# rainerzufalldererste/limg

Measured on AMD Instinct MI355X. Metric: encode Mpixels/s, 8K RGBA (limg_encode3d_test-equivalent: all 11 planes stored), higher is better.
Workload: dtype u8/i32 integer stage + f32 float stage (bit-exact vs the reference's strict SSE build)

## Files before the change

limg_amd/csrc/limg_hip_search.h:

```cpp
#ifndef LIMG_HIP_SEARCH_H
#define LIMG_HIP_SEARCH_H

#include "limg_hip_device.h"
#include "limg_search_table.h"

namespace limg_hip
{
  namespace
  {
    struct __attribute__((aligned(32))) SearchEntry { uint32_t w[8]; };
    __constant__ SearchEntry d_search_tab[LIMG_SEARCH_STATES] = LIMG_SEARCH_TABLE_INIT;

    typedef short short2_t __attribute__((ext_vector_type(2)));
    typedef unsigned short ushort2_t __attribute__((ext_vector_type(2)));
    __device__ __forceinline__ constexpr int term_bias(int factor) { return factor == 2 ? 0x2000 : 0x3000; }
    __device__ __forceinline__ int term_const(int f, int c, int lo) { return 255 - ((lo << 8) + 128) + (c < 2 ? (term_bias(f) << 8) : 0); }

    struct TrialState
    {
      uint32_t fA, fB, fC;
      uint32_t loRG, hiRG;
      int pxB, pxBlo;
      int nA[3], nB[3], nC[3];
      int mA[3], mB[3], mC[3];
      uint32_t tA_RG, tB_RG, tC_RG;
      int tA_B, tB_B, tC_B;
      uint32_t cA, cB, cC;
    };

    __device__ __forceinline__ void make_terms(const uint32_t f, const uint32_t s, const uint32_t mul, const int n[3], const int m[3], uint32_t &tRG, int &tB)
    {
      const int d = (int)mul_u24_uniform(f >> (s & 31u), mul);
      const int t0 = mad_i24(d, n[0], m[0]), t1 = mad_i24(d, n[1], m[1]), t2 = mad_i24(d, n[2], m[2]);
      tRG = __builtin_amdgcn_perm((uint32_t)t1, (uint32_t)t0, 0x06050201u);
      tB = t2 >> 8;
    }

    __device__ __forceinline__ void rebuild_A(TrialState &t, const uint32_t sA, const uint32_t mul) { make_terms(t.fA, sA, mul, t.nA, t.mA, t.tA_RG, t.tA_B); t.cA = sA; }
    __device__ __forceinline__ void rebuild_B(TrialState &t, const uint32_t sB, const uint32_t mul)
    {
      if (sB > 7) { t.tB_RG = (uint32_t)term_bias(1) * 0x10001u; t.tB_B = 0; }
      else make_terms(t.fB, sB, mul, t.nB, t.mB, t.tB_RG, t.tB_B);
      t.cB = sB;
    }
    __device__ __forceinline__ void rebuild_C(TrialState &t, const uint32_t sC, const uint32_t mul)
    {
      if (sC > 7) { t.tC_RG = (uint32_t)term_bias(2) * 0x10001u; t.tC_B = 0; }
      else make_terms(t.fC, sC, mul, t.nC, t.mC, t.tC_RG, t.tC_B);
      t.cC = sC;
    }

    template <bool FULL>
    __device__ __forceinline__ uint32_t trial_pixel_error(const TrialState &t, const bool active)
    {
      const uint32_t dRG = t.tA_RG + t.tB_RG + t.tC_RG;
      const int dBraw = t.tA_B + t.tB_B + t.tC_B;
      ushort2_t eu = __builtin_bit_cast(ushort2_t, dRG);
      eu = __builtin_elementwise_max(eu, __builtin_bit_cast(ushort2_t, t.loRG));
      eu = __builtin_elementwise_min(eu, __builtin_bit_cast(ushort2_t, t.hiRG));
      int dB = med3_i32(dBraw, t.pxBlo, t.pxB);
      const ushort2_t sq = eu * eu;
      const uint32_t sqB = (uint32_t)mul_i24(dB, dB);
      const bool low_red = sq.x < 0x4000;
      const uint32_t half = __builtin_amdgcn_udot2(sq, __builtin_bit_cast(ushort2_t, 0x00020001u), sqB, false);
      const uint32_t extra = low_red ? sqB : (__builtin_bit_cast(uint32_t, sq) & 0xFFFFu);
      uint32_t err = (half << 1) + extra;
      if (!FULL) err = active ? err : 0u;
      return err;
    }

    typedef unsigned int uint8s_t __attribute__((ext_vector_type(8)));
    __device__ __forceinline__ uint8s_t sload8(const SearchEntry *base, uint32_t byteOffset)
    {
      uint8s_t v;
      asm volatile("s_load_dwordx8 %0, %1, %2\n\ts_waitcnt lgkmcnt(0)" : "=&s"(v) : "s"(base), "s"(byteOffset) : "memory");
      return v;
    }

    template <bool FULL>
    __device__ __forceinline__ void search_fast_automaton(TrialState &t, const bool active, const uint32_t maxPixel32, const uint32_t blockLimit, uint32_t shift[3])
    {
      const SearchEntry *tab = d_search_tab;
      asm volatile("" : "+s"(tab));
      constexpr uint32_t root[8] = LIMG_SEARCH_ROOT;
      rebuild_A(t, root[0] & 31u, root[5]);
      rebuild_B(t, root[3], root[6]);
      rebuild_C(t, root[4], root[7]);
      uint8s_t e = { root[0] & ~0xE0u, root[1], root[2], root[3], root[4], root[5], root[6], root[7] };
      while (!(e[0] >> 31))
      {
        if (e[0] & 0x20u) rebuild_A(t, e[0] & 31u, e[5]);
        if (e[0] & 0x40u) rebuild_B(t, e[3], e[6]);
        if (e[0] & 0x80u) rebuild_C(t, e[4], e[7]);
        const uint32_t err = trial_pixel_error<FULL>(t, active);
        uint32_t off;
        if (__builtin_amdgcn_ballot_w64(err > maxPixel32) != 0ull) off = e[2];
        else off = (wave_sum(err) < blockLimit) ? e[1] : e[2];
        e = sload8(tab, off);
      }
      shift[0] = e[0] & 31u; shift[1] = e[3]; shift[2] = e[4];
    }

    template <bool FULL>
    __device__ __forceinline__ void search_accurate_automaton(TrialState &t, const bool active, const uint32_t maxPixel32, const uint32_t blockLimit, const uint32_t *table,
                                                              uint32_t shift[3])
    {
      const SearchEntry *tab = reinterpret_cast<const SearchEntry *>(table);
      uint32_t bestA = 0, bestB = 0, bestC = 0, minBe = 0xFFFFFFFFu;
      {
        constexpr uint32_t root[8] = LIMG_SEARCH_ROOT;
        rebuild_A(t, root[0] & 31u, root[5]);
        rebuild_B(t, root[3], root[6]);
        rebuild_C(t, root[4], root[7]);
      }
      uint8s_t e = sload8(tab, 0u);
      constexpr uint32_t rootT[8] = LIMG_SEARCH_ROOT;
      uint32_t mask = ((e[0] & 31u) != (rootT[0] & 31u) ? 1u : 0u) | (e[3] != rootT[3] ? 2u : 0u) | (e[4] != rootT[4] ? 4u : 0u);
      while (!(e[0] >> 31))
      {
        const uint32_t a = e[0] & 31u;
        if (mask & 1u) rebuild_A(t, a, e[5]);
        if (mask & 2u) rebuild_B(t, e[3], e[6]);
        if (mask & 4u) rebuild_C(t, e[4], e[7]);
        const uint32_t err = trial_pixel_error<FULL>(t, active);
        uint32_t off = e[2];
        if (__builtin_amdgcn_ballot_w64(err > maxPixel32) == 0ull)
        {
          const uint32_t be = wave_sum(err);
          if (be < blockLimit)
          {
            off = e[1];
            if (!(e[0] & 0x20u) || be < minBe) { bestA = a; bestB = e[3]; bestC = e[4]; minBe = be; }
          }
        }
        mask = off >> 24;
        e = sload8(tab, off & 0xFFFFFFu);
      }
      shift[0] = bestA; shift[1] = bestB; shift[2] = bestC;
    }

    __device__ __attribute__((noinline)) uint32_t search_generic(uint32_t px, uint32_t fA, uint32_t fB, uint32_t fC, const int16_t *rec , bool active,
                                                                 uint32_t maxPixel32, uint64_t maxBlockN, bool fast)
    {
      RecU r;
#pragma unroll
      for (int c = 0; c < 3; c++)
      {
        const int loA = rec[c], hiA = rec[4 + c], loB = rec[8 + c], hiB = rec[12 + c], loC = rec[16 + c], hiC = rec[20 + c];
        r.nA[c] = sgpr(hiA - loA); r.nB[c] = sgpr(hiB - loB); r.nC[c] = sgpr(hiC - loC);
        r.mA[c] = sgpr((int)(((uint32_t)loA << 8) + 128u)); r.mB[c] = sgpr((int)(((uint32_t)loB << 8) + 128u)); r.mC[c] = sgpr((int)(((uint32_t)loC << 8) + 128u));
      }
      uint32_t shift[3] = { 0, 0, 0 };
      auto T = [&](uint32_t a, uint32_t bb, uint32_t c, uint32_t &be2) -> bool { return trial(px, fA, fB, fC, r, a, bb, c, active, maxPixel32, maxBlockN, be2); };
      if (fast) search_fast(T, shift);
      else search_accurate(T, shift);
      return shift[0] | (shift[1] << 8) | (shift[2] << 16);
    }
  }
}

#endif
```

Before: 51070.

## Unroll hot top of fast search automaton into compile-time branch tree

```diff
diff --git a/limg_amd/csrc/limg_hip_search.h b/limg_amd/csrc/limg_hip_search.h
--- a/limg_amd/csrc/limg_hip_search.h
+++ b/limg_amd/csrc/limg_hip_search.h
@@ -77,16 +77,55 @@
       return v;
     }
 
+    struct TermSet { uint32_t rg; int b; };
+    __device__ __forceinline__ constexpr TermSet terms_shift8(int factor) { return TermSet{ (uint32_t)term_bias(factor) * 0x10001u, 0 }; }
+    template <uint32_t S, uint32_t MUL>
+    __device__ __forceinline__ TermSet hot_terms(const uint32_t f, const int n[3], const int m[3])
+    {
+      static_assert(S <= 8 && (S >= 4 || MUL == (1u << S)), "MUL is shift_mul(S)");
+      int t0, t1, t2;
+      if constexpr (S == 8) { t0 = m[0]; t1 = m[1]; t2 = m[2]; }
+      else
+      {
+        uint32_t d;
+        if constexpr (S < 4) d = f & ~((1u << S) - 1u);
+        else asm("v_mul_u32_u24 %0, %2, %1" : "=v"(d) : "v"(f >> S), "n"(MUL));
+        t0 = mad_i24((int)d, n[0], m[0]); t1 = mad_i24((int)d, n[1], m[1]); t2 = mad_i24((int)d, n[2], m[2]);
+      }
+      TermSet r;
+      r.rg = __builtin_amdgcn_perm((uint32_t)t1, (uint32_t)t0, 0x06050201u);
+      r.b = t2 >> 8;
+      return r;
+    }
+    __device__ __forceinline__ bool hot_trial(TrialState &t, const TermSet &A, const TermSet &B, const TermSet &C, const uint32_t maxPixel32, const uint32_t blockLimit)
+    {
+      t.tA_RG = A.rg; t.tA_B = A.b; t.tB_RG = B.rg; t.tB_B = B.b; t.tC_RG = C.rg; t.tC_B = C.b;
+      const uint32_t err = trial_pixel_error<true>(t, true);
+      return __builtin_amdgcn_ballot_w64(err > maxPixel32) == 0ull && wave_sum(err) < blockLimit;
+    }
+#include "limg_search_hot.h"
+
     template <bool FULL>
     __device__ __forceinline__ void search_fast_automaton(TrialState &t, const bool active, const uint32_t maxPixel32, const uint32_t blockLimit, uint32_t shift[3])
     {
       const SearchEntry *tab = d_search_tab;
-      asm volatile("" : "+s"(tab));
-      constexpr uint32_t root[8] = LIMG_SEARCH_ROOT;
-      rebuild_A(t, root[0] & 31u, root[5]);
-      rebuild_B(t, root[3], root[6]);
-      rebuild_C(t, root[4], root[7]);
-      uint8s_t e = { root[0] & ~0xE0u, root[1], root[2], root[3], root[4], root[5], root[6], root[7] };
+      uint8s_t e;
+      if constexpr (FULL)
+      {
+        uint32_t off;
+        if (search_hot(t, maxPixel32, blockLimit, shift, off)) return;
+        asm volatile("" : "+s"(tab));
+        e = sload8(tab, off);
+      }
+      else
+      {
+        asm volatile("" : "+s"(tab));
+        constexpr uint32_t root[8] = LIMG_SEARCH_ROOT;
+        rebuild_A(t, root[0] & 31u, root[5]);
+        rebuild_B(t, root[3], root[6]);
+        rebuild_C(t, root[4], root[7]);
+        e = uint8s_t{ root[0] & ~0xE0u, root[1], root[2], root[3], root[4], root[5], root[6], root[7] };
+      }
       while (!(e[0] >> 31))
       {
         if (e[0] & 0x20u) rebuild_A(t, e[0] & 31u, e[5]);
diff --git a/limg_amd/csrc/limg_search_hot.h b/limg_amd/csrc/limg_search_hot.h
--- /dev/null
+++ b/limg_amd/csrc/limg_search_hot.h
@@ -0,0 +1,260 @@
+#ifndef LIMG_SEARCH_HOT_H
+#define LIMG_SEARCH_HOT_H
+#define LIMG_SEARCH_HOT_STATES 45
+__device__ __forceinline__ bool search_hot(TrialState &t, const uint32_t maxPixel32, const uint32_t blockLimit, uint32_t shift[3], uint32_t &off)
+{
+  const TermSet tA4_0 = hot_terms<4u, 17u>(t.fA, t.nA, t.mA);
+  const TermSet tB5_0 = hot_terms<5u, 36u>(t.fB, t.nB, t.mB);
+  const TermSet tC6_0 = hot_terms<6u, 85u>(t.fC, t.nC, t.mC);
+  if (hot_trial(t, tA4_0, tB5_0, tC6_0, maxPixel32, blockLimit))
+  {
+    const TermSet tA5_1 = hot_terms<5u, 36u>(t.fA, t.nA, t.mA);
+    if (hot_trial(t, tA5_1, terms_shift8(1), terms_shift8(2), maxPixel32, blockLimit))
+    { shift[0] = 5u; shift[1] = 8u; shift[2] = 8u; return true; }
+    else
+    {
+      const TermSet tB6_3 = hot_terms<6u, 85u>(t.fB, t.nB, t.mB);
+      if (hot_trial(t, tA4_0, tB6_3, terms_shift8(2), maxPixel32, blockLimit))
+      {
+        if (hot_trial(t, tA4_0, terms_shift8(1), terms_shift8(2), maxPixel32, blockLimit))
+        { t.cA = 4u; t.cB = 8u; t.cC = 8u; off = 0x00a0u; return false; }
+        else
+        {
+          const TermSet tA6_23 = hot_terms<6u, 85u>(t.fA, t.nA, t.mA);
+          if (hot_trial(t, tA6_23, tB6_3, terms_shift8(2), maxPixel32, blockLimit))
+          {
+            if (hot_trial(t, tA6_23, terms_shift8(1), terms_shift8(2), maxPixel32, blockLimit))
+            { t.cA = 6u; t.cB = 8u; t.cC = 8u; off = 0x00c0u; return false; }
+            else
+            {
+              const TermSet tA8_25 = hot_terms<8u, 256u>(t.fA, t.nA, t.mA);
+              if (hot_trial(t, tA8_25, tB6_3, terms_shift8(2), maxPixel32, blockLimit))
+              { t.cA = 8u; t.cB = 6u; t.cC = 8u; off = 0x0180u; return false; }
+              else
+              {
+                if (hot_trial(t, tA8_25, terms_shift8(1), tC6_0, maxPixel32, blockLimit))
+                { t.cA = 8u; t.cB = 8u; t.cC = 6u; off = 0x0220u; return false; }
+                else
+                {
+                  const TermSet tB7_27 = hot_terms<7u, 255u>(t.fB, t.nB, t.mB);
+                  if (hot_trial(t, tA6_23, tB7_27, terms_shift8(2), maxPixel32, blockLimit))
+                  { t.cA = 6u; t.cB = 7u; t.cC = 8u; off = 0x0380u; return false; }
+                  else
+                  {
+                    const TermSet tA7_31 = hot_terms<7u, 255u>(t.fA, t.nA, t.mA);
+                    if (hot_trial(t, tA7_31, tB6_3, terms_shift8(2), maxPixel32, blockLimit))
+                    { t.cA = 7u; t.cB = 6u; t.cC = 8u; off = 0x0400u; return false; }
+                    else
+                    { shift[0] = 6u; shift[1] = 6u; shift[2] = 8u; return true; }
+                  }
+                }
+              }
+            }
+          }
+          else
+          {
+            if (hot_trial(t, tA6_23, terms_shift8(1), tC6_0, maxPixel32, blockLimit))
+            { t.cA = 6u; t.cB = 8u; t.cC = 6u; off = 0x0480u; return false; }
+            else
+            {
+              const TermSet tA8_47 = hot_terms<8u, 256u>(t.fA, t.nA, t.mA);
+              if (hot_trial(t, tA8_47, tB6_3, terms_shift8(2), maxPixel32, blockLimit))
+              { t.cA = 8u; t.cB = 6u; t.cC = 8u; off = 0x0180u; return false; }
+              else
+              {
+                if (hot_trial(t, tA8_47, terms_shift8(1), tC6_0, maxPixel32, blockLimit))
+                { t.cA = 8u; t.cB = 8u; t.cC = 6u; off = 0x0220u; return false; }
+                else
+                {
+                  const TermSet tB7_49 = hot_terms<7u, 255u>(t.fB, t.nB, t.mB);
+                  if (hot_trial(t, tA4_0, tB7_49, terms_shift8(2), maxPixel32, blockLimit))
+                  { t.cA = 4u; t.cB = 7u; t.cC = 8u; off = 0x0640u; return false; }
+                  else
+                  {
+                    if (hot_trial(t, tA5_1, tB6_3, terms_shift8(2), maxPixel32, blockLimit))
+                    {
+                      if (hot_trial(t, tA5_1, tB7_49, terms_shift8(2), maxPixel32, blockLimit))
+                      { shift[0] = 5u; shift[1] = 7u; shift[2] = 8u; return true; }
+                      else
+                      { shift[0] = 5u; shift[1] = 6u; shift[2] = 8u; return true; }
+                    }
+                    else
+                    { shift[0] = 4u; shift[1] = 6u; shift[2] = 8u; return true; }
+                  }
+                }
+              }
+            }
+          }
+        }
+      }
+      else
+      {
+        if (hot_trial(t, tA4_0, tB5_0, terms_shift8(2), maxPixel32, blockLimit))
+        { t.cA = 4u; t.cB = 5u; t.cC = 8u; off = 0x0740u; return false; }
+        else
+        {
+          const TermSet tB7_96 = hot_terms<7u, 255u>(t.fB, t.nB, t.mB);
+          const TermSet tC5_96 = hot_terms<5u, 36u>(t.fC, t.nC, t.mC);
+          if (hot_trial(t, tA4_0, tB7_96, tC5_96, maxPixel32, blockLimit))
+          { t.cA = 4u; t.cB = 7u; t.cC = 5u; off = 0x0c20u; return false; }
+          else
+          {
+            const TermSet tA6_112 = hot_terms<6u, 85u>(t.fA, t.nA, t.mA);
+            const TermSet tB4_112 = hot_terms<4u, 17u>(t.fB, t.nB, t.mB);
+            const TermSet tC7_112 = hot_terms<7u, 255u>(t.fC, t.nC, t.mC);
+            if (hot_trial(t, tA6_112, tB4_112, tC7_112, maxPixel32, blockLimit))
+            { t.cA = 6u; t.cB = 4u; t.cC = 7u; off = 0x0c60u; return false; }
+            else
+            {
+              const TermSet tC4_113 = hot_terms<4u, 17u>(t.fC, t.nC, t.mC);
+              if (hot_trial(t, tA6_112, tB6_3, tC4_113, maxPixel32, blockLimit))
+              { t.cA = 6u; t.cB = 6u; t.cC = 4u; off = 0x0e40u; return false; }
+              else
+              {
+                if (hot_trial(t, tA6_112, terms_shift8(1), tC6_0, maxPixel32, blockLimit))
+                { t.cA = 6u; t.cB = 8u; t.cC = 6u; off = 0x0480u; return false; }
+                else
+                {
+                  const TermSet tA8_138 = hot_terms<8u, 256u>(t.fA, t.nA, t.mA);
+                  if (hot_trial(t, tA8_138, tB6_3, terms_shift8(2), maxPixel32, blockLimit))
+                  { t.cA = 8u; t.cB = 6u; t.cC = 8u; off = 0x0180u; return false; }
+                  else
+                  {
+                    if (hot_trial(t, tA8_138, terms_shift8(1), tC6_0, maxPixel32, blockLimit))
+                    { t.cA = 8u; t.cB = 8u; t.cC = 6u; off = 0x0220u; return false; }
+                    else
+                    {
+                      if (hot_trial(t, tA4_0, tB5_0, tC7_112, maxPixel32, blockLimit))
+                      { t.cA = 4u; t.cB = 5u; t.cC = 7u; off = 0x11a0u; return false; }
+                      else
+                      {
+                        if (hot_trial(t, tA5_1, tB5_0, tC6_0, maxPixel32, blockLimit))
+                        {
+                          if (hot_trial(t, tA5_1, tB5_0, tC7_112, maxPixel32, blockLimit))
+                          { shift[0] = 5u; shift[1] = 5u; shift[2] = 7u; return true; }
+                          else
+                          { shift[0] = 5u; shift[1] = 5u; shift[2] = 6u; return true; }
+                        }
+                        else
+                        { shift[0] = 4u; shift[1] = 5u; shift[2] = 6u; return true; }
+                      }
+                    }
+                  }
+                }
+              }
+            }
+          }
+        }
+      }
+    }
+  }
+  else
+  {
+    const TermSet tA2_148 = hot_terms<2u, 4u>(t.fA, t.nA, t.mA);
+    const TermSet tB4_148 = hot_terms<4u, 17u>(t.fB, t.nB, t.mB);
+    const TermSet tC5_148 = hot_terms<5u, 36u>(t.fC, t.nC, t.mC);
+    if (hot_trial(t, tA2_148, tB4_148, tC5_148, maxPixel32, blockLimit))
+    {
+      const TermSet tC7_149 = hot_terms<7u, 255u>(t.fC, t.nC, t.mC);
+      if (hot_trial(t, tA2_148, tB4_148, tC7_149, maxPixel32, blockLimit))
+      { t.cA = 2u; t.cB = 4u; t.cC = 7u; off = 0x12c0u; return false; }
+      else
+      {
+        const TermSet tB6_378 = hot_terms<6u, 85u>(t.fB, t.nB, t.mB);
+        const TermSet tC4_378 = hot_terms<4u, 17u>(t.fC, t.nC, t.mC);
+        if (hot_trial(t, tA2_148, tB6_378, tC4_378, maxPixel32, blockLimit))
+        { t.cA = 2u; t.cB = 6u; t.cC = 4u; off = 0x2f60u; return false; }
+        else
+        {
+          if (hot_trial(t, tA2_148, terms_shift8(1), tC6_0, maxPixel32, blockLimit))
+          { t.cA = 2u; t.cB = 8u; t.cC = 6u; off = 0x18e0u; return false; }
+          else
+          {
+            const TermSet tB2_412 = hot_terms<2u, 4u>(t.fB, t.nB, t.mB);
+            if (hot_trial(t, tA4_0, tB2_412, terms_shift8(2), maxPixel32, blockLimit))
+            { t.cA = 4u; t.cB = 2u; t.cC = 8u; off = 0x2500u; return false; }
+            else
+            {
+              if (hot_trial(t, tA4_0, tB4_148, tC4_378, maxPixel32, blockLimit))
+              {
+                if (hot_trial(t, tA4_0, tB4_148, tC6_0, maxPixel32, blockLimit))
+                { t.cA = 4u; t.cB = 4u; t.cC = 6u; off = 0x2700u; return false; }
+                else
+                {
+                  if (hot_trial(t, tA4_0, tB6_378, tC4_378, maxPixel32, blockLimit))
+                  { t.cA = 4u; t.cB = 6u; t.cC = 4u; off = 0x2a40u; return false; }
+                  else
+                  {
+                    if (hot_trial(t, tA4_0, terms_shift8(1), tC6_0, maxPixel32, blockLimit))
+                    { t.cA = 4u; t.cB = 8u; t.cC = 6u; off = 0x1460u; return false; }
+                    else
+                    {
+                      const TermSet tA6_417 = hot_terms<6u, 85u>(t.fA, t.nA, t.mA);
+                      if (hot_trial(t, tA6_417, tB4_148, terms_shift8(2), maxPixel32, blockLimit))
+                      { t.cA = 6u; t.cB = 4u; t.cC = 8u; off = 0x1620u; return false; }
+                      else
+                      {
+                        if (hot_trial(t, tA6_417, tB6_378, tC4_378, maxPixel32, blockLimit))
+                        { t.cA = 6u; t.cB = 6u; t.cC = 4u; off = 0x0e40u; return false; }
+                        else
+                        {
+                          if (hot_trial(t, tA6_417, terms_shift8(1), tC6_0, maxPixel32, blockLimit))
+                          { t.cA = 6u; t.cB = 8u; t.cC = 6u; off = 0x0480u; return false; }
+                          else
+                          {
+                            const TermSet tA8_420 = hot_terms<8u, 256u>(t.fA, t.nA, t.mA);
+                            if (hot_trial(t, tA8_420, tB6_378, terms_shift8(2), maxPixel32, blockLimit))
+                            { t.cA = 8u; t.cB = 6u; t.cC = 8u; off = 0x0180u; return false; }
+                            else
+                            {
+                              if (hot_trial(t, tA8_420, terms_shift8(1), tC6_0, maxPixel32, blockLimit))
+                              { t.cA = 8u; t.cB = 8u; t.cC = 6u; off = 0x0220u; return false; }
+                              else
+                              {
+                                if (hot_trial(t, tA4_0, tB4_148, tC5_148, maxPixel32, blockLimit))
+                                {
+                                  if (hot_trial(t, tA4_0, tB5_0, tC5_148, maxPixel32, blockLimit))
+                                  {
+                                    const TermSet tA5_424 = hot_terms<5u, 36u>(t.fA, t.nA, t.mA);
+                                    if (hot_trial(t, tA5_424, tB5_0, tC5_148, maxPixel32, blockLimit))
+                                    { shift[0] = 5u; shift[1] = 5u; shift[2] = 5u; return true; }
+                                    else
+                                    { shift[0] = 4u; shift[1] = 5u; shift[2] = 5u; return true; }
+                                  }
+                                  else
+                                  {
+                                    const TermSet tA5_427 = hot_terms<5u, 36u>(t.fA, t.nA, t.mA);
+                                    if (hot_trial(t, tA5_427, tB4_148, tC5_148, maxPixel32, blockLimit))
+                                    { t.cA = 5u; t.cB = 4u; t.cC = 5u; off = 0x3580u; return false; }
+                                    else
+                                    {
+                                      if (hot_trial(t, tA5_427, tB5_0, tC4_378, maxPixel32, blockLimit))
+                                      { t.cA = 5u; t.cB = 5u; t.cC = 4u; off = 0x35e0u; return false; }
+                                      else
+                                      { shift[0] = 4u; shift[1] = 4u; shift[2] = 5u; return true; }
+                                    }
+                                  }
+                                }
+                                else
+                                { t.cA = 4u; t.cB = 4u; t.cC = 5u; off = 0x3640u; return false; }
+                              }
+                            }
+                          }
+                        }
+                      }
+                    }
+                  }
+                }
+              }
+              else
+              { t.cA = 4u; t.cB = 4u; t.cC = 4u; off = 0x3780u; return false; }
+            }
+          }
+        }
+      }
+    }
+    else
+    { t.cA = 2u; t.cB = 4u; t.cC = 5u; off = 0x3880u; return false; }
+  }
+}
+#endif
```

Result: faster. 55550 (median of 6 runs) (+8.8%).
